# bcgsc/ntJoin

Hardware: AMD Instinct MI355X
Metric: Gbp/s minimizer-sketch+graph-build (k=32,w=1000) (higher is better)
Workload: dtype u64

## Files before the change

ntjoin_amd/csrc/graph.hip:

```cpp
#include <algorithm>
#include <cstdlib>
#include <cstring>
#include <system_error>
#include <thread>

#include "mxg_internal.h"
#include "scan_kernels.h"

namespace mxg {

static constexpr uint64_t HT_EMPTY = 0xFFFFFFFFFFFFFFFFull;
static constexpr uint32_t NONE32 = 0xFFFFFFFFu;

struct Slot {
    unsigned long long key;
    uint32_t nseen, ndup;
};

__device__ __forceinline__ uint32_t ht_slot(Slot *tab, uint32_t mask, uint32_t cap, uint64_t key)
{
    if (key == HT_EMPTY) return cap;
    uint32_t s = (uint32_t)((key * 0x9E3779B97F4A7C15ull) >> 32) & mask;
    while (true) {
        unsigned long long cur = tab[s].key;
// ... 574 lines not shown
    }
    if (n_all > skew_lim) {
        __shared__ unsigned long long skey[PJ_IPB];
        __shared__ uint32_t sitem[PJ_IPB];
        __shared__ uint8_t sasm[PJ_IPB];
        __shared__ uint32_t stab[PJ_IPB];
        __shared__ uint32_t sdup[PJ_IPB / 32];
        for (uint32_t q = threadIdx.x; q < PJ_IPB; q += PJ_BT) stab[q] = 0xFFFFFFFFu;
        for (uint32_t q = threadIdx.x; q < PJ_IPB / 32; q += PJ_BT) sdup[q] = 0;
#pragma unroll
        for (uint32_t u = 0; u < U; ++u) {
            const uint32_t q = u * PJ_BT + threadIdx.x;
            skey[q] = ((unsigned long long)rec[u].y << 32) | rec[u].x;
            sitem[q] = rec[u].z;
            sasm[q] = (uint8_t)(rec[u].w & 0xFFu);
        }
        __syncthreads();
#pragma unroll
        for (uint32_t u = 0; u < U; ++u) {
            if (!((live >> u) & 1u)) continue;
            const uint32_t q = u * PJ_BT + threadIdx.x;
            const unsigned long long key = skey[q];
            const uint32_t a = rec[u].w & 0xFFu;
            uint32_t hsl = (uint32_t)(((key + a) * 0x9E3779B97F4A7C15ull) >> 40) & (2u * PJ_IPB - 1u);
            uint32_t rep = q;
            for (;;) {
                const uint32_t sft = (hsl & 1u) * 16u;
                const uint32_t word = stab[hsl >> 1], cur = (word >> sft) & 0xFFFFu;
                if (cur == 0xFFFFu) {
                    const uint32_t want = (word & ~(0xFFFFu << sft)) | (q << sft);
                    if (atomicCAS(&stab[hsl >> 1], word, want) == word) break;
                    continue;
                }
                if (skey[cur] == key && sasm[cur] == a) {
                    rep = cur;
                    break;
                }
                hsl = (hsl + 1u) & (2u * PJ_IPB - 1u);
            }
            if (rep != q) {
                atomicOr(&sdup[rep >> 5], 1u << (rep & 31u));
                p.slot[a][rec[u].z] = (sitem[rep] << 3) | PJ_VERDICT_REF;
                live &= ~(1u << u);
            }
        }
        __syncthreads();
#pragma unroll
        for (uint32_t u = 0; u < U; ++u) {
            const uint32_t q = u * PJ_BT + threadIdx.x;
            if ((sdup[q >> 5] >> (q & 31u)) & 1u) rec[u].w |= PJ_REC_DUP;
        }
    }
    for (uint32_t b = threadIdx.x; b <= pmask; b += PJ_BT) hist[b] = 0;
    __syncthreads();
#pragma unroll
    for (uint32_t u = 0; u < U; ++u)
        if ((live >> u) & 1u) atomicAdd(&hist[pj_part(((uint64_t)rec[u].y << 32) | rec[u].x, pmask)], 1u);
    __syncthreads();
    const uint32_t P = pmask + 1, per = P >= PJ_BT ? P / PJ_BT : 1u, b0 = threadIdx.x * per;
    uint32_t cn = 0;
    if (b0 < P)
        for (uint32_t u = 0; u < per; ++u) cn += hist[b0 + u];
    uint32_t run = block_exclusive<PJ_BT / 64>(cn, sh);
    uint32_t *row = M + ((size_t)c * rows2 + row_j) * (P + 1);
    if (b0 < P)
        for (uint32_t u = 0; u < per; ++u) {
            const uint32_t cb = hist[b0 + u];
            start[b0 + u] = run;
            row[b0 + u] = run;
            hist[b0 + u] = 0;
            run += cb;
        }
    if (threadIdx.x == 0) row[P] = sh[255];
    __syncthreads();
#pragma unroll
    for (uint32_t u = 0; u < U; ++u) {
        if (!((live >> u) & 1u)) continue;
        const uint32_t b = pj_part(((uint64_t)rec[u].y << 32) | rec[u].x, pmask);
        const uint32_t pos = (uint32_t)base + start[b] + atomicAdd(&hist[b], 1u);
        recs2[pos] = rec[u];
    }
}

__global__ __launch_bounds__(256) void k_flags_pj(const AsmSet p, uint32_t *cnt, uint32_t *sup, uint64_t *mask0)
{
    const uint32_t a = asm_of_block(p, blockIdx.x);
    const uint32_t i = (blockIdx.x - p.bstart[a]) * 256u + threadIdx.x;
    bool sh = false;
    {
        const bool in = i < asm_n(p, a);
        const uint32_t lane = threadIdx.x & 63u;
        const uint64_t fb = p.fol[blockIdx.x * 4u + (threadIdx.x >> 6)];
        const uint32_t v_raw = in ? p.slot[a][i] : 0u;
        const bool isf = (fb >> lane) & 1ull;
        uint32_t v = isf ? 0u : v_raw;
        bool other = isf;
        if ((v & 7u) == PJ_VERDICT_REF) {
            v = p.slot[a][v >> 3];
            other = true;
        }
        const uint32_t lead = 63u - (uint32_t)__clzll(~fb & ((2ull << lane) - 1ull));
        const uint32_t vl = __shfl(v, lead);
        if (isf) v = vl;
        if (other) v &= MXG_MX_INALL;
        if (in) {
            sh = (v & MXG_MX_SHARED) != 0;
            p.flags[a][i] = (uint8_t)(v & 7u);
            p.shared[a][i] = sh ? 1 : 0;
        }
    }
    const uint64_t bm = __ballot(sh);
    if (a == 0 && (threadIdx.x & 63u) == 0) mask0[(blockIdx.x - p.bstart[0]) * 4u + (threadIdx.x >> 6)] = bm;
    const uint32_t c = (uint32_t)__syncthreads_count(sh ? 1 : 0);
    if (threadIdx.x == 0) count_publish(cnt + p.bstart[a], sup + sup_start(p, a), blockIdx.x - p.bstart[a], c);
}

struct VertexParams {
    const uint8_t *shared;
    const uint32_t *cnt, *sup;
    uint64_t *n_shared;
    const uint32_t *slot;
    const uint64_t *hash;
    const uint32_t *pos, *rec;
    uint32_t n;
    const uint32_t *n_ptr;
    uint32_t first;
    uint32_t *vid;
    uint64_t *vhash;
    uint32_t *vpos, *vrec;
    uint32_t *fv, *frec;
    uint32_t *ivid;
};

__global__ __launch_bounds__(256) void k_vertices(const VertexParams p)
{
    __shared__ uint32_t sh[256];
    const uint32_t i = blockIdx.x * 256u + threadIdx.x;
    const bool f = i < (p.n_ptr ? min(*p.n_ptr, p.n) : p.n) && p.shared[i];
    __shared__ uint32_t sh_before;
    if (threadIdx.x < 64) {
        const uint32_t bef = count_prefix(p.cnt, p.sup, blockIdx.x);
        if (threadIdx.x == 0) sh_before = bef;
        if (blockIdx.x + 1 == gridDim.x) {
            const uint32_t all = count_prefix(p.cnt, p.sup, (p.n + 255u) / 256u);
            if (threadIdx.x == 0) *p.n_shared = all;
        }
    }
    __syncthreads();
    const uint32_t r = sh_before + block_exclusive_256(f ? 1u : 0u, sh);
    if (!f) return;
    const uint32_t s = p.slot[i];
    uint32_t v;
    if (p.first) {
        v = r;
        p.vid[s] = v;
        p.vhash[v] = p.hash[i];
    } else {
        v = p.vid[s];
    }
    const uint32_t rec = p.rec[i];
    p.vpos[v] = p.pos[i];
    p.vrec[v] = rec;
    if (p.ivid) p.ivid[i] = v;
    p.fv[r] = v;
    p.frec[r] = rec;
}

__global__ __launch_bounds__(256) void k_block_prefix(const uint32_t *__restrict__ cnt, const uint32_t *__restrict__ sup, uint32_t n,
                                                      uint32_t *__restrict__ out)
{
    __shared__ uint32_t sh[256];
    __shared__ uint32_t sh_before;
    const uint32_t e = blockIdx.x * 256u + threadIdx.x;
    const uint32_t c = e < n ? cnt[e] : 0u;
    if (threadIdx.x < 64) {
        const uint32_t bef = count_prefix(cnt, sup, blockIdx.x * 256u);
        if (threadIdx.x == 0) sh_before = bef;
    }
    __syncthreads();
    const uint32_t r = sh_before + block_exclusive_256(c, sh);
    if (e < n) out[e] = r;
}

struct VertexPjParams {
    AsmSet as;
    const uint32_t *pos[MXG_MAX_ASSEMBLIES], *rec[MXG_MAX_ASSEMBLIES];
    const uint32_t *cnt, *sup;
    uint64_t *n_shared;
    const uint64_t *mask0;
    const uint32_t *bpref0;
    uint64_t *vhash;
    uint32_t *vpos, *vrec, *fv, *frec;
    uint32_t nvs;
    uint32_t *ivid[MXG_MAX_ASSEMBLIES];
};

__global__ __launch_bounds__(256) void k_vertices_pj(const VertexPjParams p)
{
    __shared__ uint32_t sh[256];
    __shared__ uint32_t sh_before;
    const uint32_t a = asm_of_block(p.as, blockIdx.x);
    const uint32_t blk = blockIdx.x - p.as.bstart[a], nblk = p.as.bstart[a + 1] - p.as.bstart[a];
    const uint32_t i = blk * 256u + threadIdx.x;
    const bool in = i < asm_n(p.as, a);
    const uint8_t shf = in ? p.as.shared[a][i] : (uint8_t)0;
    const uint32_t vw = in && a ? p.as.slot[a][i] : 0u;
    const uint32_t rec = in ? p.rec[a][i] : 0u, pos = in ? p.pos[a][i] : 0u;
    const uint64_t hsh = in && !a ? p.as.hash[0][i] : 0ull;
    const bool f = shf != 0;
    uint32_t v0 = 0;
    if (f && a) {
        const uint32_t i0 = vw >> 3, w = i0 >> 6;
        const uint64_t *m = p.mask0 + (w & ~3u);
        v0 = p.bpref0[i0 >> 8] + (uint32_t)__popcll(p.mask0[w] & ((1ull << (i0 & 63u)) - 1ull));
        for (uint32_t q = 0; q < (w & 3u); ++q) v0 += (uint32_t)__popcll(m[q]);
    }
    if (threadIdx.x < 64) {
        const uint32_t *cnt = p.cnt + p.as.bstart[a], *sup = p.sup + sup_start(p.as, a);
        const uint32_t bef = count_prefix(cnt, sup, blk);
        if (threadIdx.x == 0) sh_before = bef;
        if (blk + 1 == nblk) {
            const uint32_t all = count_prefix(cnt, sup, nblk);
            if (threadIdx.x == 0) p.n_shared[a] = all;
        }
    }
    __syncthreads();
    const uint32_t r = sh_before + block_exclusive_256(f ? 1u : 0u, sh);
    if (in && p.ivid[a]) p.ivid[a][i] = f ? (a ? v0 : r) : 0xFFFFFFFFu;
    if (!f) return;
    const uint32_t v = a ? v0 : r;
    if (!a) p.vhash[v] = hsh;
    const size_t o = (size_t)a * p.nvs;
    p.vpos[o + v] = pos;
    p.vrec[o + v] = rec;
    p.fv[o + r] = v;
    p.frec[o + r] = rec;
}

__global__ __launch_bounds__(256) void k_adjacency(const uint32_t *__restrict__ fv0, const uint32_t *__restrict__ frec0,
                                                   const uint64_t *__restrict__ nv_ptr, uint2 *__restrict__ adj0, uint32_t stride)
{
    const uint32_t nv = (uint32_t)*nv_ptr;
    const size_t o = (size_t)blockIdx.y * stride;
    const uint32_t *fv = fv0 + o, *frec = frec0 + o;
    const uint32_t r = blockIdx.x * 256u + threadIdx.x;
    if (r >= nv) return;
    const uint32_t rec = frec[r];
    const uint32_t nx = (r + 1 < nv && frec[r + 1] == rec) ? fv[r + 1] : NONE32;
    const uint32_t pv = (r > 0 && frec[r - 1] == rec) ? fv[r - 1] : NONE32;
    adj0[o + fv[r]] = make_uint2(nx, pv);
}

struct EdgeParams {
    const uint32_t *fv;
    const uint2 *adj;
    const uint64_t *nv_ptr;
    uint32_t nv, n_asm;
    uint8_t *eflag;
    uint32_t *bsum;
    uint32_t *bsuper;
    uint64_t *n_edges;
    uint64_t *host_ctl;
    uint32_t *eu, *ev, *esup;
    double *ew;
    double weights[MXG_MAX_ASSEMBLIES];
};

__device__ __forceinline__ uint32_t edge_mask(const EdgeParams &p, uint32_t u, uint32_t v)
{
    uint32_t m = 0;
    for (uint32_t b = 0; b < p.n_asm; ++b) {
        const uint2 q = p.adj[(size_t)b * p.nv + u];
        if (q.x == v || q.y == v) m |= 1u << b;
    }
    return m;
}

__global__ __launch_bounds__(256) void k_edge_flags(const EdgeParams p)
{
    uint64_t item = (uint64_t)blockIdx.x * 256u + threadIdx.x;
    uint8_t f = 0;
    if (item < (uint64_t)p.n_asm * p.nv) {
        uint32_t a = (uint32_t)(item / p.nv);
        uint32_t r = (uint32_t)(item % p.nv);
        if (r < (uint32_t)*p.nv_ptr) {
            const uint32_t u = p.fv[item];
            uint32_t v, m = 0;
            if (p.n_asm <= 4u) {
                uint2 q[4];
#pragma unroll
                for (uint32_t b = 0; b < 4u; ++b) q[b] = b < p.n_asm ? p.adj[(size_t)b * p.nv + u] : make_uint2(NONE32, NONE32);
                v = a == 0 ? q[0].x : a == 1 ? q[1].x : a == 2 ? q[2].x : q[3].x;
#pragma unroll
                for (uint32_t b = 0; b < 4u; ++b)
                    if (b < p.n_asm && (q[b].x == v || q[b].y == v)) m |= 1u << b;
            } else {
                v = p.adj[(size_t)a * p.nv + u].x;
                if (v != NONE32) m = edge_mask(p, u, v);
            }
            if (v != NONE32) f = ((uint32_t)__builtin_ctz(m) == a) ? (p.n_asm <= 8u ? (uint8_t)m : (uint8_t)1) : (uint8_t)0;
        }
        p.eflag[item] = f;
    }
    const uint32_t c = (uint32_t)__syncthreads_count(f);
    if (threadIdx.x == 0) count_publish(p.bsum, p.bsuper, blockIdx.x, c);
}

__global__ __launch_bounds__(256) void k_edges(const EdgeParams p, uint32_t n_items)
{
    __shared__ uint32_t sh[256];
    const uint32_t item = blockIdx.x * 256u + threadIdx.x;
    const uint32_t fb = item < n_items ? p.eflag[item] : 0u;
    const bool f = fb != 0;
    uint32_t u = 0, v = 0, m = 0;
    double wsum = 0.0;
    if (f) {
        const uint32_t a = item / p.nv;
        u = p.fv[item];
        v = p.adj[(size_t)a * p.nv + u].x;
// ... 12 lines not shown
                p.host_ctl[32] = all;
            }
            if (threadIdx.x < p.n_asm) p.host_ctl[threadIdx.x] = p.nv_ptr[threadIdx.x];
        }
    }
    __syncthreads();
    const uint32_t e = sh_before + block_exclusive_256(f ? 1u : 0u, sh);
    if (!f) return;
    p.eu[e] = u;
    p.ev[e] = v;
    p.esup[e] = m;
    p.ew[e] = wsum;
}

__global__ __launch_bounds__(256) void k_apply_msgs(const uint4 *__restrict__ msgs, uint64_t n, uint32_t stride, uint32_t *adj)
{
    const uint64_t i = (uint64_t)blockIdx.x * 256u + threadIdx.x;
    if (i >= n) return;
    const uint4 m = msgs[i];
    adj[((size_t)(m.x & 255u) * stride + m.y) * 2u + ((m.x >> 8) ? 1u : 0u)] = m.z;
}

__global__ __launch_bounds__(256) void k_iota_rows(uint32_t *a, uint32_t stride)
{
    const uint32_t i = blockIdx.x * 256u + threadIdx.x;
    if (i < stride) a[(size_t)blockIdx.y * stride + i] = i;
}

template <class T>
static int d2h(mxg_handle *h, std::vector<T> &dst, const void *src, size_t n)
{
    dst.resize(n);
    if (n) MXG_HIP(h, hipMemcpyAsync(dst.data(), src, n * sizeof(T), hipMemcpyDeviceToHost, h->stream));
    return MXG_OK;
}

__global__ __launch_bounds__(256) void k_count_unique(const uint8_t *__restrict__ flags, uint32_t n, unsigned long long *counter)
{
    uint32_t i = blockIdx.x * 256u + threadIdx.x;
    bool u = i < n && (flags[i] & MXG_MX_UNIQUE);
    uint64_t m = __ballot(u);
    if ((threadIdx.x & 63u) == 0 && m) atomicAdd(counter, (unsigned long long)__popcll(m));
}

enum CtlWord : uint32_t {
    CTL_SHARED = 0,
    CTL_EDGES = 32,
    CTL_UNIQUE = 33,
    CTL_PJ_FAIL = 34,
    CTL_WORDS = 40,
};
static_assert(CTL_SHARED + MXG_MAX_ASSEMBLIES <= CTL_EDGES, "the per-assembly counts end before the other words");

static int build_graph_impl(mxg_handle *h, const GraphCall &c, bool global_table);

int build_graph(mxg_handle *h, const GraphCall &c)
{
    h->stat_graph_join = 0;
    uint64_t how = 0;
    JoinLearnt &learnt = h->pj_learnt;
    if (!c.gb) {
        uint64_t n_mx[MXG_MAX_ASSEMBLIES];
        const uint32_t n = (uint32_t)std::min<size_t>(h->asms.size(), MXG_MAX_ASSEMBLIES);
        for (uint32_t a = 0; a < n; ++a) n_mx[a] = h->asms[a]->n_mx;
        learnt.sketches_are(JoinLearnt::signature(n, n_mx));
    }
    int rc = build_graph_impl(h, c, learnt.overflowed);
    if (rc == RC_RETRY_PJ) {
        how |= MXG_JOIN_RESIZED;
        rc = build_graph_impl(h, c, false);
    }
    if (rc == RC_RETRY_PJ) rc = RC_RETRY_GLOBAL;
    if (rc == RC_RETRY_GLOBAL) {
        how |= MXG_JOIN_GAVE_UP;
        learnt.gave_up();
        rc = build_graph_impl(h, c, true);
    }
    h->stat_graph_join |= how;
    return rc;
}

struct JoinPlan : JoinShape {
    uint32_t pj_force_fail = 0;
    uint64_t *pj_mask0 = nullptr;
    uint32_t *pj_bpref0 = nullptr;
    AsmSet as_all;
    uint32_t n_fsup = 0, n_esup = 0;
    uint32_t *fsup = nullptr, *esup = nullptr, *cnt = nullptr;
    uint32_t *M = nullptr, *cursor = nullptr;
    uint4 *recs1 = nullptr, *recs2 = nullptr;
    PjSubCaps sc;
    size_t clear_words = 0;
};

static int plan_join(mxg_handle *h, int mode, const GraphBounds *gb, bool global_table, bool split, JoinPlan &pl)
{
    const uint32_t A = (uint32_t)h->asms.size();
    if (A == 0) return set_err(h, MXG_EINVAL, "mxg_build_graph: no assemblies");
    if (A > MXG_MAX_ASSEMBLIES) return set_err(h, MXG_ELIMIT, "at most %d assemblies", MXG_MAX_ASSEMBLIES);
    pl = JoinPlan();
    JoinRequest rq;
    rq.A = A;
    for (uint32_t ai = 0; ai < A; ++ai) {
        Assembly *a = h->asms[ai];
        if (!gb && !a->has_sketch) return set_err(h, MXG_EINVAL, "assembly '%s' has no sketch (call mxg_sketch)", a->name.c_str());
        rq.n_of[ai] = gb ? gb->n_bound[ai] : a->n_mx;
    }
    rq.mode = mode;
    rq.bounds = gb != nullptr;
    rq.global_table = global_table;
    rq.split = split;
    const char *join_env = knob_raw(h, "MXG_GRAPH_JOIN");
    rq.join_global = join_env && !strcmp(join_env, "global");
    rq.force_two_level = knob_u64(h, "MXG_PJ_TWO_LEVEL", 0) != 0;
    switch (join_shape(rq, h->pj_learnt, pl)) {
    case JS_TOO_MANY_MINIMIZERS: return set_err(h, MXG_ELIMIT, "too many minimizers for one table (%llu)", (unsigned long long)pl.N);
    case JS_TOO_MANY_ITEMS: return set_err(h, MXG_ELIMIT, "graph too large for 32-bit item indices");
    case JS_OK: break;
    }
    pl.pj_force_fail = knob_u64(h, "MXG_PJ_FORCE_FAIL", 0) ? 1u : 0u;
    pl.sc.n_sub = pl.n_sub;
    for (uint32_t a = 0; a < MXG_MAX_ASSEMBLIES; ++a) pl.sc.cap[a] = pl.sub_cap[a];
    const uint64_t *const n_of = pl.n_of;
    const uint32_t nb = pl.nb, P = pl.P, P1 = pl.P1;

    if (!pl.pj) MXG_HIP(h, h->g_keys.ensure(((size_t)pl.cap + 1) * sizeof(Slot)));
    const size_t nb0 = pl.nb0, nb_all = nb;
    MXG_HIP(h, h->g_vid.ensure(pl.pj ? (nb0 + nb_all) * 4 * 8 + nb0 * 4 + 64 : ((size_t)pl.cap + 1) * 4));
    pl.pj_mask0 = h->g_vid.as<uint64_t>();
    uint64_t *const pj_fol = pl.pj_mask0 + nb0 * 4;
    pl.pj_bpref0 = reinterpret_cast<uint32_t *>(pj_fol + nb_all * 4);
    MXG_HIP(h, h->g_ctl.ensure(CTL_WORDS * 8));

    AsmSet &as_all = pl.as_all;
    as_all.n_asm = A;
    as_all.full = pl.full;
    as_all.fol = pl.pj ? pj_fol : nullptr;
    for (uint32_t a = 0; a < A; ++a) {
        Assembly *as = h->asms[a];
        MXG_HIP(h, as->d_slot.ensure(std::max<uint64_t>(n_of[a] * 4, 16)));
        MXG_HIP(h, as->d_flags.ensure(std::max<uint64_t>(n_of[a], 16)));
        MXG_HIP(h, as->d_shared.ensure(std::max<uint64_t>(n_of[a], 16)));
        as_all.n[a] = (uint32_t)n_of[a];
        as_all.n_ptr[a] = gb ? gb->n_ptr[a] : nullptr;
        as_all.hash[a] = as->d_hash.as<uint64_t>();
        as_all.slot[a] = as->d_slot.as<uint32_t>();
        as_all.flags[a] = as->d_flags.as<uint8_t>();
        as_all.shared[a] = as->d_shared.as<uint8_t>();
    }
    for (uint32_t a = A; a < MXG_MAX_ASSEMBLIES; ++a) {
        as_all.n[a] = 0;
        as_all.n_ptr[a] = nullptr;
        as_all.hash[a] = nullptr;
        as_all.slot[a] = nullptr;
        as_all.flags[a] = as_all.shared[a] = nullptr;
    }
    std::copy(pl.bstart, pl.bstart + MXG_MAX_ASSEMBLIES + 1, as_all.bstart);
    pl.n_fsup = ((nb >> SUP_SHIFT) + A + 1) * SUP_STRIDE;
    pl.n_esup = sup_words(pl.e_blocks);
    MXG_HIP(h, h->g_cnt.ensure(((size_t)pl.n_fsup + pl.n_esup + pl.n_cur + nb) * 4 + 64));
    pl.fsup = h->g_cnt.as<uint32_t>();
    pl.esup = pl.fsup + pl.n_fsup;
    pl.cnt = pl.esup + pl.n_esup + pl.n_cur;
    pl.clear_words = (size_t)pl.n_fsup + pl.n_esup + pl.n_cur;
    const bool resume = mode == GRAPH_DG_EDGES || mode == GRAPH_DG_EDGES_APPLIED;
    if (nb && !resume && pl.pj && pl.two_level) {
        const size_t n_recs = (size_t)P1 * pl.cap1;
        MXG_HIP(h, h->g_part.ensure((size_t)P1 * pl.rows2 * (P + 1) * 4 + (size_t)P1 * PJ1_CS * 4));
        MXG_HIP(h, h->g_keys.ensure(n_recs * sizeof(uint4)));
        MXG_HIP(h, h->g_recs1.ensure(n_recs * sizeof(uint4)));
        pl.M = h->g_part.as<uint32_t>();
        pl.cursor = pl.n_cur ? pl.esup + pl.n_esup : pl.M + (size_t)P1 * pl.rows2 * (P + 1);
        pl.recs1 = h->g_recs1.as<uint4>();
        pl.recs2 = h->g_keys.as<uint4>();
    }
    return MXG_OK;
}

static void launch_partition(mxg_handle *h, const JoinPlan &pl, uint32_t a_lo, uint32_t a_hi, hipStream_t st, uint32_t n_sup_clear)
{
    const uint32_t blk_lo = pl.as_all.bstart[a_lo], blk_hi = pl.as_all.bstart[a_hi];
    const uint32_t n_rows1 = (blk_hi - blk_lo + PJ_IPB / 256 - 1) / (PJ_IPB / 256);
    PjSub sub{1u, 0u, 0u, pl.cap1};
    uint32_t skew_lim = (uint32_t)std::min<uint64_t>(pl.N / pl.P1 + pl.N / pl.P1 / 32 + 2048, 0xFFFFFFFFull);
    if (pl.split) {
        sub = PjSub{pl.A, a_lo, pl.sub_off[a_lo], pl.sub_cap[a_lo]};
        skew_lim = pl.skew_lim[a_lo];
    }
    if (n_rows1)
        hipLaunchKernelGGL(k_pj1_scatter, dim3(n_rows1), dim3(PJ_BT), (size_t)pl.P1 * 8, st, pl.as_all, blk_lo, blk_hi, pl.P1 - 1, pl.cap1,
                           pl.cursor, pl.recs1, pl.fsup, n_sup_clear, sub);
    hipLaunchKernelGGL(k_pj2_bucket, dim3(sub.cap / PJ_IPB, pl.P1), dim3(PJ_BT), (size_t)pl.P * 8, st, pl.as_all, pl.recs1, pl.cursor, pl.cap1,
                       pl.rows2, pl.P - 1, pl.M, pl.recs2, knob_u64(h, "MXG_PJ_SKEW", 0) ? 0u : skew_lim, sub);
}

static int ev_pair(mxg_handle *h, hipEvent_t *a, hipEvent_t *b)
{
    while (h->ev_pool.size() < h->ev_used + 2) {
        hipEvent_t e;
        MXG_HIP(h, hipEventCreate(&e));
        h->ev_pool.push_back(e);
    }
    *a = h->ev_pool[h->ev_used];
    *b = h->ev_pool[h->ev_used + 1];
    h->ev_used += 2;
    h->ev_spans.push_back(TimedSpan{*a, *b, 0, false, 5});
    return MXG_OK;
}

int graph_plan_early(mxg_handle *h, const GraphBounds &gb, bool *early)
{
    *early = false;
    h->pj_early_done = 0;
    if (knob_u64(h, "MXG_PJ_EARLY", 1) == 0) return MXG_OK;
    MXG_HIP(h, hipSetDevice(h->device));
    if (!h->pj_plan) h->pj_plan = new JoinPlan;
    JoinPlan &pl = *h->pj_plan;
    const std::string err_before = h->err;
    if (plan_join(h, GRAPH_FULL, &gb, h->pj_learnt.overflowed, true, pl) != MXG_OK || !(pl.pj && pl.two_level && pl.split && pl.nb)) {
        pl = JoinPlan();
        h->err = err_before;
        return MXG_OK;
    }
    MXG_HIP(h, hipMemsetAsync(pl.fsup, 0, pl.clear_words * 4, h->stream));
    if (!h->ev_plan) MXG_HIP(h, hipEventCreateWithFlags(&h->ev_plan, hipEventDisableTiming));
    MXG_HIP(h, hipEventRecord(h->ev_plan, h->stream));
    *early = true;
    return MXG_OK;
}

int graph_partition_early(mxg_handle *h, uint32_t a, hipStream_t st)
// ... 14 lines not shown
    if (fine) MXG_HIP(h, hipEventRecord(e1, st));
    ++h->pj_early_done;
    return MXG_OK;
}

void graph_drop_plan(mxg_handle *h)
{
    delete h->pj_plan;
    h->pj_plan = nullptr;
}

static int take_or_make_plan(mxg_handle *h, const GraphCall &c, bool global_table, JoinPlan &own, const JoinPlan **plan)
{
    const JoinPlan *ep = h->pj_plan;
    bool early = ep && ep->split && h->pj_early_done != 0 && h->pj_early_done == ep->A && c.gb && c.mode == GRAPH_FULL && !global_table &&
                 ep->A == h->asms.size();
    for (uint32_t a = 0; early && a < ep->A; ++a) early = c.gb->n_bound[a] == ep->n_of[a] && c.gb->n_ptr[a] == ep->as_all.n_ptr[a];
    h->pj_early_done = 0;
    *plan = early ? ep : &own;
    if (early) return MXG_OK;
    const int rc = plan_join(h, c.mode, c.gb, global_table, false, own);
    if (rc != MXG_OK && c.mode != GRAPH_DG_EDGES && c.mode != GRAPH_DG_EDGES_APPLIED)
        for (Assembly *a : h->asms) a->flags_valid = a->flags_on_host = false;
    return rc;
}

struct GraphStage {
    mxg_handle *const h;
    const GraphCall &c;
    const JoinPlan &pl;
    const bool early;
    const bool resume;
    const bool fine, timing;
    Graph &g;
    uint64_t *ctl = nullptr, *hctl = nullptr;
    uint64_t *pj_fail = nullptr;

    GraphStage(mxg_handle *h_, const GraphCall &c_, const JoinPlan &pl_, bool early_)
        : h(h_), c(c_), pl(pl_), early(early_), resume(c_.mode == GRAPH_DG_EDGES || c_.mode == GRAPH_DG_EDGES_APPLIED),
          fine((h_->cfg.flags & MXG_FLAG_TIMING_FINE) != 0 && c_.mode == GRAPH_FULL), timing((h_->cfg.flags & MXG_FLAG_TIMING) != 0 || fine),
          g(h_->graph)
    {
    }
    bool joins() const { return pl.nb && !resume; }
    size_t anv() const { return (size_t)pl.A * pl.nvs; }

    int begin()
    {
        for (uint32_t ai = 0; ai < pl.A; ++ai) {
            Assembly *a = h->asms[ai];
            if (!resume) a->flags_on_host = false;
            a->flags_valid = true;
        }
        if (!resume) g = Graph();
        g.n_asm = pl.A;
        if (fine && !h->ev_g[0]) {
            MXG_HIP(h, hipEventCreate(&h->ev_g[0]));
            MXG_HIP(h, hipEventCreate(&h->ev_g[1]));
        }
        if (timing) MXG_HIP(h, hipEventRecord(h->ev0, h->stream));
        if (!resume)
            h->stat_graph_join = (pl.pj ? (pl.two_level ? MXG_JOIN_LDS_TWO_LEVEL : MXG_JOIN_LDS) : MXG_JOIN_GLOBAL) | (early ? MXG_JOIN_EARLY : 0);
        if (!pl.pj && !resume) MXG_HIP(h, hipMemsetAsync(h->g_keys.p, 0xFF, ((size_t)pl.cap + 1) * sizeof(Slot), h->stream));
        ctl = h->g_ctl.as<uint64_t>();
        if (!h->pinned_gctl) MXG_HIP(h, hipHostMalloc((void **)&h->pinned_gctl, CTL_WORDS * 8));
        hctl = h->pinned_gctl;
        memset(hctl, 0, CTL_WORDS * 8);
        pj_fail = pl.dg_pj ? dg_pj_fail_word(h) : hctl + CTL_PJ_FAIL;
        return MXG_OK;
    }

    void launch_join(uint4 *recs, uint32_t *M, uint32_t n_parts, uint32_t n_rows, const uint32_t *cursor)
    {
        const bool narrow = pl.A <= 16;
        const uint32_t cap1 = cursor ? pl.cap1 : 0u, rows2 = cursor ? pl.rows2 : 0u;
        const uint64_t pipe_blocks = cursor ? knob_u64(h, "MXG_PJ_PIPE", 1024) : 0;
        if (pipe_blocks && rows2 <= 256)
            hipLaunchKernelGGL(narrow ? k_pj_join_pipe<true> : k_pj_join_pipe<false>, dim3((uint32_t)std::min<uint64_t>(pipe_blocks, n_parts)),
                               dim3(256), 0, h->stream, recs, M, pl.P, n_parts, pj_fail, pl.pj_force_fail, cursor, cap1, rows2, pl.as_all, pl.sc);
        else
            hipLaunchKernelGGL(narrow ? k_pj_join<true> : k_pj_join<false>, dim3(n_parts), dim3(256), 0, h->stream, recs, M, pl.P, n_rows,
                               pj_fail, pl.pj_force_fail, cursor, cap1, rows2, pl.as_all, pl.sc);
    }
    int join_two_level()
    {
        if (!early) {
            MXG_HIP(h, hipMemsetAsync(pl.cursor, 0, (size_t)pl.P1 * PJ1_CS * 4, h->stream));
            launch_partition(h, pl, 0, pl.A, h->stream, pl.n_fsup + pl.n_esup);
        }
        launch_join(pl.recs2, pl.M, pl.P1 * pl.P, 0u, pl.cursor);
        hipLaunchKernelGGL(k_flags_pj, dim3(pl.nb), dim3(256), 0, h->stream, pl.as_all, pl.cnt, pl.fsup, pl.pj_mask0);
        return MXG_OK;
    }
    int join_one_level()
    {
        const uint32_t n_rows = (pl.nb + PJ_IPB / 256 - 1) / (PJ_IPB / 256);
        MXG_HIP(h, h->g_part.ensure((size_t)n_rows * (pl.P + 1) * 4));
        MXG_HIP(h, h->g_keys.ensure((size_t)n_rows * PJ_IPB * sizeof(uint4)));
        uint32_t *M = h->g_part.as<uint32_t>();
        uint4 *recs = h->g_keys.as<uint4>();
        hipLaunchKernelGGL(k_pj_bucket, dim3(n_rows), dim3(PJ_BT), (size_t)pl.P * 8, h->stream, pl.as_all, pl.nb, pl.P - 1, M, recs, pl.fsup,
                           pl.n_fsup + pl.n_esup);
        launch_join(recs, M, pl.P, n_rows, nullptr);
        hipLaunchKernelGGL(k_flags_pj, dim3(pl.nb), dim3(256), 0, h->stream, pl.as_all, pl.cnt, pl.fsup, pl.pj_mask0);
        return MXG_OK;
    }
    int join_global()
    {
        hipLaunchKernelGGL(k_insert, dim3(pl.nb), dim3(256), 0, h->stream, pl.as_all, h->g_keys.as<Slot>(), pl.mask, pl.cap, pl.fsup,
                           pl.n_fsup + pl.n_esup);
        hipLaunchKernelGGL(k_flags, dim3(pl.nb), dim3(256), 0, h->stream, pl.as_all, h->g_keys.as<Slot>(), pl.cnt, pl.fsup);
        return MXG_OK;
    }
    int mark(hipEvent_t ev)
    {
        MXG_HIP(h, hipGetLastError());
        if (fine) MXG_HIP(h, hipEventRecord(ev, h->stream));
        return MXG_OK;
    }

    int vertex_arrays()
    {
        MXG_HIP(h, h->g_vhash.ensure(pl.nvs * 8));
        MXG_HIP(h, h->g_vpos.ensure(anv() * 4));
        MXG_HIP(h, h->g_vrec.ensure(anv() * 4));
        MXG_HIP(h, h->g_fv.ensure(anv() * 4));
        MXG_HIP(h, h->g_frec.ensure(anv() * 4));
        MXG_HIP(h, h->g_nxt.ensure(2 * anv() * 4));
        if (c.mode == GRAPH_DG_EDGES) MXG_HIP(h, hipMemsetAsync(h->g_nxt.p, 0xFF, 2 * anv() * 4, h->stream));
        return MXG_OK;
    }
    int item_vids(uint32_t a, uint32_t **ivid)
    {
        *ivid = nullptr;
        if (c.mode != GRAPH_DG_VERTICES) return MXG_OK;
        MXG_HIP(h, h->asms[a]->d_ivid.ensure((size_t)pl.n_of[a] * 4 + 16));
        *ivid = h->asms[a]->d_ivid.as<uint32_t>();
        return MXG_OK;
    }
    int fill(VertexPjParams &vp)
    {
        vp.as = pl.as_all;
        for (uint32_t a = 0; a < MXG_MAX_ASSEMBLIES; ++a) {
            vp.pos[a] = a < pl.A ? h->asms[a]->d_pos.as<uint32_t>() : nullptr;
            vp.rec[a] = a < pl.A ? h->asms[a]->d_rec.as<uint32_t>() : nullptr;
            vp.ivid[a] = nullptr;
            int rc;
            if (a < pl.A && (rc = item_vids(a, &vp.ivid[a])) != MXG_OK) return rc;
        }
        vp.cnt = pl.cnt;
        vp.sup = pl.fsup;
        vp.n_shared = ctl + CTL_SHARED;
        vp.mask0 = pl.pj_mask0;
        vp.bpref0 = pl.pj_bpref0;
        vp.vhash = h->g_vhash.as<uint64_t>();
        vp.vpos = h->g_vpos.as<uint32_t>();
        vp.vrec = h->g_vrec.as<uint32_t>();
        vp.fv = h->g_fv.as<uint32_t>();
        vp.frec = h->g_frec.as<uint32_t>();
        vp.nvs = (uint32_t)pl.nvs;
        return MXG_OK;
    }
    int vertices_pj()
    {
        VertexPjParams vp;
        const int rc = fill(vp);
        if (rc != MXG_OK) return rc;
        hipLaunchKernelGGL(k_block_prefix, dim3((uint32_t)((pl.nb0 + 255) / 256)), dim3(256), 0, h->stream, pl.cnt + pl.as_all.bstart[0],
                           pl.fsup + sup_start(pl.as_all, 0), (uint32_t)pl.nb0, pl.pj_bpref0);
        hipLaunchKernelGGL(k_vertices_pj, dim3(pl.nb), dim3(256), 0, h->stream, vp);
        return MXG_OK;
    }
    int fill(VertexParams &vp, uint32_t a)
    {
        Assembly *as = h->asms[a];
        const size_t row = (size_t)a * pl.nvs;
        vp.shared = as->d_shared.as<uint8_t>();
        vp.cnt = pl.cnt + pl.as_all.bstart[a];
        vp.sup = pl.fsup + sup_start(pl.as_all, a);
        vp.n_shared = ctl + CTL_SHARED + a;
        vp.slot = as->d_slot.as<uint32_t>();
        vp.hash = as->d_hash.as<uint64_t>();
        vp.pos = as->d_pos.as<uint32_t>();
        vp.rec = as->d_rec.as<uint32_t>();
        vp.n = (uint32_t)pl.n_of[a];
        vp.n_ptr = c.gb ? c.gb->n_ptr[a] : nullptr;
        vp.first = a == 0;
        vp.vid = h->g_vid.as<uint32_t>();
        vp.vhash = h->g_vhash.as<uint64_t>();
        vp.vpos = h->g_vpos.as<uint32_t>() + row;
        vp.vrec = h->g_vrec.as<uint32_t>() + row;
        vp.fv = h->g_fv.as<uint32_t>() + row;
        vp.frec = h->g_frec.as<uint32_t>() + row;
        return item_vids(a, &vp.ivid);
    }
    int vertices_global()
    {
        for (uint32_t a = 0; a < pl.A; ++a) {
            VertexParams vp;
            const int rc = fill(vp, a);
            if (rc != MXG_OK) return rc;
            if (vp.ivid) MXG_HIP(h, hipMemsetAsync(vp.ivid, 0xFF, (size_t)vp.n * 4, h->stream));
            hipLaunchKernelGGL(k_vertices, dim3((vp.n + 255) / 256), dim3(256), 0, h->stream, vp);
        }
        return MXG_OK;
    }
    int hand_back_vertices()
    {
        g.nv_stride = pl.nvs;
        if (!c.d_n_vertices) return MXG_OK;
        if (pl.nvs > 0) MXG_HIP(h, hipMemcpyAsync(c.d_n_vertices, ctl + CTL_SHARED, 8, hipMemcpyDeviceToDevice, h->stream));
        else MXG_HIP(h, hipMemsetAsync(c.d_n_vertices, 0, 8, h->stream));
        return MXG_OK;
    }

    void adjacency_own()
    {
        hipLaunchKernelGGL(k_adjacency, dim3((uint32_t)((pl.nvs + 255) / 256), pl.A), dim3(256), 0, h->stream, h->g_fv.as<uint32_t>(),
                           h->g_frec.as<uint32_t>(), ctl + CTL_SHARED, h->g_nxt.as<uint2>(), (uint32_t)pl.nvs);
    }
    void adjacency_of_owner()
    {
        if (c.n_msgs && c.mode == GRAPH_DG_EDGES)
            hipLaunchKernelGGL(k_apply_msgs, dim3((uint32_t)((c.n_msgs + 255) / 256)), dim3(256), 0, h->stream,
                               static_cast<const uint4 *>(c.d_msgs), c.n_msgs, (uint32_t)pl.nvs, h->g_nxt.as<uint32_t>());
        hipLaunchKernelGGL(k_iota_rows, dim3((uint32_t)((pl.nvs + 255) / 256), pl.A), dim3(256), 0, h->stream, h->g_fv.as<uint32_t>(),
                           (uint32_t)pl.nvs);
    }

    void fill(EdgeParams &ep)
    {
        ep.fv = h->g_fv.as<uint32_t>();
        ep.adj = h->g_nxt.as<uint2>();
        ep.nv_ptr = ctl + CTL_SHARED;
        ep.nv = (uint32_t)pl.nvs;
        ep.n_asm = pl.A;
        ep.eflag = h->g_eflag.as<uint8_t>();
        ep.bsum = h->g_ebs.as<uint32_t>();
        ep.bsuper = pl.esup;
        ep.n_edges = ctl + CTL_EDGES;
        ep.host_ctl = hctl;
        ep.eu = h->g_eu.as<uint32_t>();
        ep.ev = h->g_ev.as<uint32_t>();
        ep.esup = h->g_esup.as<uint32_t>();
        ep.ew = h->g_ew.as<double>();
        for (uint32_t a = 0; a < MXG_MAX_ASSEMBLIES; ++a) ep.weights[a] = a < pl.A ? h->asms[a]->weight : 0.0;
    }
    int edges()
    {
        const uint32_t n_items = pl.n_items;
        MXG_HIP(h, h->g_eflag.ensure(n_items));
        MXG_HIP(h, h->g_ebs.ensure((size_t)pl.e_blocks * 4 + 64));
        MXG_HIP(h, h->g_eu.ensure((size_t)n_items * 4));
        MXG_HIP(h, h->g_ev.ensure((size_t)n_items * 4));
        MXG_HIP(h, h->g_esup.ensure((size_t)n_items * 4));
        MXG_HIP(h, h->g_ew.ensure((size_t)n_items * 8));
        EdgeParams ep;
        fill(ep);
        hipLaunchKernelGGL(k_edge_flags, dim3(pl.e_blocks), dim3(256), 0, h->stream, ep);
        hipLaunchKernelGGL(k_edges, dim3(pl.e_blocks), dim3(256), 0, h->stream, ep, n_items);
        MXG_HIP(h, hipGetLastError());
        return MXG_OK;
    }

    int sync_and_verdict()
    {
        if (timing) MXG_HIP(h, hipEventRecord(h->ev1, h->stream));
        MXG_HIP(h, stream_wait(h->stream));
        if (!pl.pj || !hctl[CTL_PJ_FAIL]) return MXG_OK;
        if (!pl.two_level || pl.pj_force_fail) return RC_RETRY_GLOBAL;
        std::vector<uint32_t> cur((size_t)pl.P1 * pl.n_sub * PJ1_CS);
        MXG_HIP(h, hipMemcpy(cur.data(), pl.cursor, cur.size() * 4, hipMemcpyDeviceToHost));
        return join_overflow_verdict(pl, cur.data(), h->pj_learnt);
    }
    int results()
    {
        const uint64_t nv = hctl[CTL_SHARED];
        for (uint32_t a = 1; a < pl.A; ++a)
            if (hctl[CTL_SHARED + a] != nv)
                return set_err(h, MXG_EDEVICE, "internal error: shared-minimizer counts differ between assemblies (%llu vs %llu)",
                               (unsigned long long)hctl[CTL_SHARED + a], (unsigned long long)nv);
        g.nv = nv;
        g.nv_stride = pl.nvs;
        g.ne = pl.nvs > 0 ? hctl[CTL_EDGES] : 0;
        h->stat_unique = ~0ull;
        if (timing) {
            float ms = 0;
            MXG_HIP(h, hipEventElapsedTime(&ms, h->ev0, h->ev1));
            h->tm.ms_graph += ms;
            if (fine && pl.nvs > 0) {
                float a = 0, b = 0, c3 = 0;
                MXG_HIP(h, hipEventElapsedTime(&a, h->ev0, h->ev_g[0]));
                MXG_HIP(h, hipEventElapsedTime(&b, h->ev_g[0], h->ev_g[1]));
                MXG_HIP(h, hipEventElapsedTime(&c3, h->ev_g[1], h->ev1));
                h->tm.ms_join += a;
                h->tm.ms_vertices += b;
                h->tm.ms_edges += c3;
            }
        }
        g.valid = true;
        g.host_valid = false;
        return MXG_OK;
    }
};

static int build_graph_impl(mxg_handle *h, const GraphCall &c, bool global_table)
{
    MXG_HIP(h, hipSetDevice(h->device));
    JoinPlan own;
    const JoinPlan *plan = nullptr;
    int rc = take_or_make_plan(h, c, global_table, own, &plan);
    if (rc != MXG_OK) return rc;
    const JoinPlan &pl = *plan;
    GraphStage s(h, c, pl, plan != &own);
    if ((rc = s.begin()) != MXG_OK) return rc;
    if (s.joins() && (rc = pl.pj ? (pl.two_level ? s.join_two_level() : s.join_one_level()) : s.join_global()) != MXG_OK) return rc;
    if ((rc = s.mark(h->ev_g[0])) != MXG_OK) return rc;
    if (pl.nvs > 0) {
        if ((rc = s.vertex_arrays()) != MXG_OK) return rc;
        if (!s.resume && (rc = pl.pj ? s.vertices_pj() : s.vertices_global()) != MXG_OK) return rc;
    }
    if (c.mode == GRAPH_DG_VERTICES) return s.hand_back_vertices();
    if (pl.nvs > 0) {
        if (c.mode == GRAPH_FULL) s.adjacency_own();
        else s.adjacency_of_owner();
        if ((rc = s.mark(h->ev_g[1])) != MXG_OK) return rc;
        if ((rc = s.edges()) != MXG_OK) return rc;
    }
    if ((rc = s.sync_and_verdict()) != MXG_OK) return rc;
    return s.results();
}

int graph_to_host(mxg_handle *h)
{
    Graph &g = h->graph;
    if (!g.valid) return set_err(h, MXG_EINVAL, "call mxg_build_graph first");
    if (g.host_valid) return MXG_OK;
    MXG_HIP(h, hipSetDevice(h->device));
    const size_t anv = (size_t)g.n_asm * g.nv;
    int rc;
    {
        std::vector<std::thread> th;
        auto sized = [](auto &v, size_t n) {
            try {
                v.resize(n);
            } catch (const std::bad_alloc &) {
            }
        };
        try {
            th.emplace_back([&] { sized(g.vhash, g.nv); });
            th.emplace_back([&] { sized(g.vpos, anv); });
            th.emplace_back([&] { sized(g.vrec, anv); });
            th.emplace_back([&] { sized(g.eu, g.ne); });
            th.emplace_back([&] { sized(g.ev, g.ne); });
            th.emplace_back([&] { sized(g.esup, g.ne); });
            sized(g.ew, g.ne);
        } catch (const std::system_error &) {
        }
        for (auto &t : th) t.join();
    }
    if ((rc = d2h(h, g.vhash, h->g_vhash.p, g.nv)) != MXG_OK) return rc;
    g.vpos.resize(anv);
    g.vrec.resize(anv);
    for (uint32_t a = 0; a < g.n_asm && g.nv; ++a) {
        MXG_HIP(h, hipMemcpyAsync(g.vpos.data() + (size_t)a * g.nv, h->g_vpos.as<uint32_t>() + (size_t)a * g.nv_stride,
                                  g.nv * 4, hipMemcpyDeviceToHost, h->stream));
        MXG_HIP(h, hipMemcpyAsync(g.vrec.data() + (size_t)a * g.nv, h->g_vrec.as<uint32_t>() + (size_t)a * g.nv_stride,
                                  g.nv * 4, hipMemcpyDeviceToHost, h->stream));
    }
    if ((rc = d2h(h, g.eu, h->g_eu.p, g.ne)) != MXG_OK) return rc;
    if ((rc = d2h(h, g.ev, h->g_ev.p, g.ne)) != MXG_OK) return rc;
    if ((rc = d2h(h, g.esup, h->g_esup.p, g.ne)) != MXG_OK) return rc;
    if ((rc = d2h(h, g.ew, h->g_ew.p, g.ne)) != MXG_OK) return rc;
    MXG_HIP(h, hipStreamSynchronize(h->stream));
    g.host_valid = true;
    return MXG_OK;
}

int flags_to_host(mxg_handle *h, Assembly *a)
{
    if (!a->flags_valid) return set_err(h, MXG_EINVAL, "call mxg_build_graph first");
    if (a->flags_on_host) return MXG_OK;
    MXG_HIP(h, hipSetDevice(h->device));
    int rc = d2h(h, a->h_flags, a->d_flags.p, a->n_mx);
    if (rc != MXG_OK) return rc;
    MXG_HIP(h, hipStreamSynchronize(h->stream));
    a->flags_on_host = true;
    return MXG_OK;
}

}
```

Baseline: 2504.

## Fuse adjacency into vertex kernel and widen flags kernel to four items per thread

The flags kernel now handles four minimizers per thread with vectorized slot loads and packed flag stores. It builds per-block shared masks for every assembly, so the per-item shared byte array is no longer written. The vertex kernel reads sharedness from those masks. In full-graph mode it also computes next/previous neighbours in shared memory, using cross-block searches for the nearest shared item, which removes the separate adjacency kernel and the frec array. This cuts memory traffic and a kernel launch, at the cost of more complex boundary logic and extra wave work in the vertex kernel.

```diff
diff --git a/ntjoin_amd/csrc/graph.hip b/ntjoin_amd/csrc/graph.hip
--- a/ntjoin_amd/csrc/graph.hip
+++ b/ntjoin_amd/csrc/graph.hip
@@ -680,37 +680,104 @@
     }
 }
 
-__global__ __launch_bounds__(256) void k_flags_pj(const AsmSet p, uint32_t *cnt, uint32_t *sup, uint64_t *mask0)
-{
-    const uint32_t a = asm_of_block(p, blockIdx.x);
-    const uint32_t i = (blockIdx.x - p.bstart[a]) * 256u + threadIdx.x;
-    bool sh = false;
-    {
-        const bool in = i < asm_n(p, a);
-        const uint32_t lane = threadIdx.x & 63u;
-        const uint64_t fb = p.fol[blockIdx.x * 4u + (threadIdx.x >> 6)];
-        const uint32_t v_raw = in ? p.slot[a][i] : 0u;
-        const bool isf = (fb >> lane) & 1ull;
-        uint32_t v = isf ? 0u : v_raw;
-        bool other = isf;
-        if ((v & 7u) == PJ_VERDICT_REF) {
-            v = p.slot[a][v >> 3];
-            other = true;
-        }
-        const uint32_t lead = 63u - (uint32_t)__clzll(~fb & ((2ull << lane) - 1ull));
-        const uint32_t vl = __shfl(v, lead);
-        if (isf) v = vl;
-        if (other) v &= MXG_MX_INALL;
-        if (in) {
-            sh = (v & MXG_MX_SHARED) != 0;
-            p.flags[a][i] = (uint8_t)(v & 7u);
-            p.shared[a][i] = sh ? 1 : 0;
-        }
-    }
-    const uint64_t bm = __ballot(sh);
-    if (a == 0 && (threadIdx.x & 63u) == 0) mask0[(blockIdx.x - p.bstart[0]) * 4u + (threadIdx.x >> 6)] = bm;
-    const uint32_t c = (uint32_t)__syncthreads_count(sh ? 1 : 0);
-    if (threadIdx.x == 0) count_publish(cnt + p.bstart[a], sup + sup_start(p, a), blockIdx.x - p.bstart[a], c);
+__device__ __forceinline__ uint64_t spread16_by4(uint64_t x)
+{
+    x &= 0xFFFFull;
+    x = (x | (x << 24)) & 0x000000FF000000FFull;
+    x = (x | (x << 12)) & 0x000F000F000F000Full;
+    x = (x | (x << 6)) & 0x0303030303030303ull;
+    x = (x | (x << 3)) & 0x1111111111111111ull;
+    return x;
+}
+template <uint32_t IPT>
+__host__ __device__ __forceinline__ uint32_t flags_pj_tiles(const AsmSet &p, uint32_t a)
+{
+    return (p.bstart[a + 1] - p.bstart[a] + IPT - 1u) / IPT;
+}
+
+template <uint32_t IPT>
+__global__ __launch_bounds__(256) void k_flags_pj(const AsmSet p, uint32_t *cnt, uint32_t *sup, uint64_t *mask)
+{
+    static_assert(IPT == 1 || IPT == 4, "a thread's minimizers lie in one follower word; a 256-block is a wave (4) or the block (1)");
+    __shared__ uint32_t lv[256 * IPT];
+    uint32_t a = 0, tile = blockIdx.x;
+    for (;;) {
+        const uint32_t nt = flags_pj_tiles<IPT>(p, a);
+        if (a + 1 >= p.n_asm || tile < nt) break;
+        tile -= nt;
+        ++a;
+    }
+    const uint32_t nblk = p.bstart[a + 1] - p.bstart[a], n = asm_n(p, a);
+    const uint32_t t0 = threadIdx.x * IPT, i0 = tile * (256u * IPT) + t0;
+    const uint32_t blk = i0 >> 8, bit0 = i0 & 63u;
+    const bool blk_in = blk < nblk;
+    const size_t w = ((size_t)p.bstart[a] + blk) * 4u + ((i0 >> 6) & 3u);
+    const uint64_t fb = blk_in ? p.fol[w] : 0ull;
+    uint32_t v[IPT];
+    bool whole = false;
+    if constexpr (IPT == 4) {
+        whole = i0 + 4u <= n;
+        if (whole) {
+            const uint4 q = *reinterpret_cast<const uint4 *>(p.slot[a] + i0);
+            v[0] = q.x, v[1] = q.y, v[2] = q.z, v[3] = q.w;
+        }
+    }
+    if (!whole) {
+#pragma unroll
+        for (uint32_t j = 0; j < IPT; ++j) v[j] = i0 + j < n ? p.slot[a][i0 + j] : 0u;
+    }
+    uint32_t other = 0;
+#pragma unroll
+    for (uint32_t j = 0; j < IPT; ++j) {
+        const bool isf = (fb >> (bit0 + j)) & 1ull;
+        if (isf) {
+            v[j] = 0u;
+            other |= 1u << j;
+        }
+        if ((v[j] & 7u) == PJ_VERDICT_REF) {
+            v[j] = p.slot[a][v[j] >> 3];
+            other |= 1u << j;
+        }
+        lv[t0 + j] = v[j];
+    }
+    __syncthreads();
+    uint32_t fl = 0, shm = 0;
+#pragma unroll
+    for (uint32_t j = 0; j < IPT; ++j) {
+        const uint32_t bit = bit0 + j;
+        if ((fb >> bit) & 1ull)
+            v[j] = lv[(t0 & ~63u) + 63u - (uint32_t)__clzll(~fb & ((2ull << bit) - 1ull))];
+        if ((other >> j) & 1u) v[j] &= MXG_MX_INALL;
+        if (i0 + j < n) {
+            fl |= (v[j] & 7u) << (8u * j);
+            shm |= ((v[j] & MXG_MX_SHARED) ? 1u : 0u) << j;
+        }
+    }
+    if (whole) {
+        *reinterpret_cast<uint32_t *>(p.flags[a] + i0) = fl;
+    } else {
+#pragma unroll
+        for (uint32_t j = 0; j < IPT; ++j)
+            if (i0 + j < n) p.flags[a][i0 + j] = (uint8_t)(fl >> (8u * j));
+    }
+    const uint32_t lane = threadIdx.x & 63u;
+    if constexpr (IPT == 4) {
+        uint64_t mw = 0;
+        uint32_t c = 0;
+#pragma unroll
+        for (uint32_t j = 0; j < IPT; ++j) {
+            const uint64_t b = __ballot((shm >> j) & 1u);
+            mw |= spread16_by4(b >> (lane & 48u)) << j;
+            c += (uint32_t)__popcll(b);
+        }
+        if (blk_in && (lane & 15u) == 0) mask[w] = mw;
+        if (blk_in && lane == 0) count_publish(cnt + p.bstart[a], sup + sup_start(p, a), blk, c);
+    } else {
+        const uint64_t bm = __ballot(shm & 1u);
+        if (lane == 0) mask[w] = bm;
+        const uint32_t c = (uint32_t)__syncthreads_count(shm & 1u);
+        if (threadIdx.x == 0) count_publish(cnt + p.bstart[a], sup + sup_start(p, a), blk, c);
+    }
 }
 
 struct VertexParams {
@@ -785,54 +852,115 @@
     const uint32_t *pos[MXG_MAX_ASSEMBLIES], *rec[MXG_MAX_ASSEMBLIES];
     const uint32_t *cnt, *sup;
     uint64_t *n_shared;
-    const uint64_t *mask0;
+    const uint64_t *mask;
     const uint32_t *bpref0;
     uint64_t *vhash;
-    uint32_t *vpos, *vrec, *fv, *frec;
+    uint32_t *vpos, *vrec, *fv;
+    uint2 *adj;
     uint32_t nvs;
     uint32_t *ivid[MXG_MAX_ASSEMBLIES];
 };
 
+__device__ __forceinline__ uint32_t pj_vertex_of(const VertexPjParams &p, uint32_t i0)
+{
+    const uint32_t w = i0 >> 6;
+    const uint64_t *m = p.mask + (w & ~3u);
+    uint32_t v0 = p.bpref0[i0 >> 8] + (uint32_t)__popcll(p.mask[w] & ((1ull << (i0 & 63u)) - 1ull));
+    for (uint32_t q = 0; q < (w & 3u); ++q) v0 += (uint32_t)__popcll(m[q]);
+    return v0;
+}
+
+__device__ __forceinline__ uint32_t pj_shared_before(const uint32_t *cnt, const uint64_t *mask, uint32_t blk, bool far)
+{
+    const uint32_t lane = threadIdx.x & 63u;
+    for (uint32_t hi = blk; hi > 0; hi = hi > 64u ? hi - 64u : 0u) {
+        const uint64_t some = __ballot(lane < hi && cnt[hi - 1u - (lane < hi ? lane : 0u)] != 0u);
+        if (some) {
+            const uint32_t b = hi - 1u - (uint32_t)__builtin_ctzll(some);
+            const uint64_t m = mask[(size_t)b * 4u + (lane & 3u)];
+            const uint32_t q = 31u - (uint32_t)__builtin_clz((uint32_t)__ballot(m != 0ull) & 15u);
+            return b * 256u + q * 64u + 63u - (uint32_t)__clzll(__shfl(m, (int)q));
+        }
+        if (!far) break;
+    }
+    return NONE32;
+}
+__device__ __forceinline__ uint32_t pj_shared_after(const uint32_t *cnt, const uint64_t *mask, uint32_t blk, uint32_t nblk, bool far)
+{
+    const uint32_t lane = threadIdx.x & 63u;
+    for (uint32_t lo = blk + 1u; lo < nblk; lo += 64u) {
+        const uint64_t some = __ballot(lo + lane < nblk && cnt[lo + lane < nblk ? lo + lane : lo] != 0u);
+        if (some) {
+            const uint32_t b = lo + (uint32_t)__builtin_ctzll(some);
+            const uint64_t m = mask[(size_t)b * 4u + (lane & 3u)];
+            const uint32_t q = (uint32_t)__builtin_ctz((uint32_t)__ballot(m != 0ull) & 15u);
+            return b * 256u + q * 64u + (uint32_t)__builtin_ctzll(__shfl(m, (int)q));
+        }
+        if (!far) break;
+    }
+    return NONE32;
+}
+
 __global__ __launch_bounds__(256) void k_vertices_pj(const VertexPjParams p)
 {
     __shared__ uint32_t sh[256];
     __shared__ uint32_t sh_before;
+    __shared__ uint32_t nb_v[258], nb_rec[258];
     const uint32_t a = asm_of_block(p.as, blockIdx.x);
     const uint32_t blk = blockIdx.x - p.as.bstart[a], nblk = p.as.bstart[a + 1] - p.as.bstart[a];
-    const uint32_t i = blk * 256u + threadIdx.x;
+    const uint32_t i = blk * 256u + threadIdx.x, wave = threadIdx.x >> 6, lane = threadIdx.x & 63u;
     const bool in = i < asm_n(p.as, a);
-    const uint8_t shf = in ? p.as.shared[a][i] : (uint8_t)0;
+    const bool f = (p.mask[(size_t)blockIdx.x * 4u + wave] >> lane) & 1ull;
     const uint32_t vw = in && a ? p.as.slot[a][i] : 0u;
     const uint32_t rec = in ? p.rec[a][i] : 0u, pos = in ? p.pos[a][i] : 0u;
     const uint64_t hsh = in && !a ? p.as.hash[0][i] : 0ull;
-    const bool f = shf != 0;
-    uint32_t v0 = 0;
-    if (f && a) {
-        const uint32_t i0 = vw >> 3, w = i0 >> 6;
-        const uint64_t *m = p.mask0 + (w & ~3u);
-        v0 = p.bpref0[i0 >> 8] + (uint32_t)__popcll(p.mask0[w] & ((1ull << (i0 & 63u)) - 1ull));
-        for (uint32_t q = 0; q < (w & 3u); ++q) v0 += (uint32_t)__popcll(m[q]);
-    }
-    if (threadIdx.x < 64) {
-        const uint32_t *cnt = p.cnt + p.as.bstart[a], *sup = p.sup + sup_start(p.as, a);
+    const uint32_t v0 = f && a ? pj_vertex_of(p, vw >> 3) : 0u;
+    const uint32_t *cnt = p.cnt + p.as.bstart[a];
+    uint32_t out_v = NONE32, out_rec = 0, out_i = NONE32;
+    if (wave == 0) {
+        const uint32_t *sup = p.sup + sup_start(p.as, a);
         const uint32_t bef = count_prefix(cnt, sup, blk);
         if (threadIdx.x == 0) sh_before = bef;
         if (blk + 1 == nblk) {
             const uint32_t all = count_prefix(cnt, sup, nblk);
             if (threadIdx.x == 0) p.n_shared[a] = all;
         }
+    } else if (wave <= 2 && p.adj) {
+        const uint64_t *mask = p.mask + (size_t)p.as.bstart[a] * 4u;
+        const bool far = cnt[blk] != 0u;
+        out_i = wave == 1 ? pj_shared_before(cnt, mask, blk, far) : pj_shared_after(cnt, mask, blk, nblk, far);
+        if (out_i != NONE32) {
+            out_rec = p.rec[a][out_i];
+            if (a) out_v = pj_vertex_of(p, p.as.slot[a][out_i] >> 3);
+        }
     }
     __syncthreads();
-    const uint32_t r = sh_before + block_exclusive_256(f ? 1u : 0u, sh);
-    if (in && p.ivid[a]) p.ivid[a][i] = f ? (a ? v0 : r) : 0xFFFFFFFFu;
+    const uint32_t q = block_exclusive_256(f ? 1u : 0u, sh), r = sh_before + q;
+    const uint32_t v = a ? v0 : r;
+    if (in && p.ivid[a]) p.ivid[a][i] = f ? v : 0xFFFFFFFFu;
+    const size_t o = (size_t)a * p.nvs;
+    if (f) {
+        if (!a) p.vhash[v] = hsh;
+        p.vpos[o + v] = pos;
+        p.vrec[o + v] = rec;
+        p.fv[o + r] = v;
+    }
+    if (!p.adj) return;
+    const uint32_t total = sh[255];
+    if (f) {
+        nb_v[1u + q] = v;
+        nb_rec[1u + q] = rec;
+    }
+    if ((wave == 1 || wave == 2) && lane == 0) {
+        const uint32_t at = wave == 1 ? 0u : 1u + total;
+        nb_v[at] = out_i == NONE32 ? NONE32 : a ? out_v : wave == 1 ? sh_before - 1u : sh_before + total;
+        nb_rec[at] = out_rec;
+    }
+    __syncthreads();
     if (!f) return;
-    const uint32_t v = a ? v0 : r;
-    if (!a) p.vhash[v] = hsh;
-    const size_t o = (size_t)a * p.nvs;
-    p.vpos[o + v] = pos;
-    p.vrec[o + v] = rec;
-    p.fv[o + r] = v;
-    p.frec[o + r] = rec;
+    const uint32_t nx = nb_rec[2u + q] == rec ? nb_v[2u + q] : NONE32;
+    const uint32_t pv = nb_rec[q] == rec ? nb_v[q] : NONE32;
+    p.adj[o + v] = make_uint2(nx, pv);
 }
 
 __global__ __launch_bounds__(256) void k_adjacency(const uint32_t *__restrict__ fv0, const uint32_t *__restrict__ frec0,
@@ -1011,7 +1139,7 @@
 
 struct JoinPlan : JoinShape {
     uint32_t pj_force_fail = 0;
-    uint64_t *pj_mask0 = nullptr;
+    uint64_t *pj_mask = nullptr;
     uint32_t *pj_bpref0 = nullptr;
     AsmSet as_all;
     uint32_t n_fsup = 0, n_esup = 0;
@@ -1055,9 +1183,9 @@
 
     if (!pl.pj) MXG_HIP(h, h->g_keys.ensure(((size_t)pl.cap + 1) * sizeof(Slot)));
     const size_t nb0 = pl.nb0, nb_all = nb;
-    MXG_HIP(h, h->g_vid.ensure(pl.pj ? (nb0 + nb_all) * 4 * 8 + nb0 * 4 + 64 : ((size_t)pl.cap + 1) * 4));
-    pl.pj_mask0 = h->g_vid.as<uint64_t>();
-    uint64_t *const pj_fol = pl.pj_mask0 + nb0 * 4;
+    MXG_HIP(h, h->g_vid.ensure(pl.pj ? (nb_all + nb_all) * 4 * 8 + nb0 * 4 + 64 : ((size_t)pl.cap + 1) * 4));
+    pl.pj_mask = h->g_vid.as<uint64_t>();
+    uint64_t *const pj_fol = pl.pj_mask + nb_all * 4;
     pl.pj_bpref0 = reinterpret_cast<uint32_t *>(pj_fol + nb_all * 4);
     MXG_HIP(h, h->g_ctl.ensure(CTL_WORDS * 8));
 
@@ -1069,13 +1197,13 @@
         Assembly *as = h->asms[a];
         MXG_HIP(h, as->d_slot.ensure(std::max<uint64_t>(n_of[a] * 4, 16)));
         MXG_HIP(h, as->d_flags.ensure(std::max<uint64_t>(n_of[a], 16)));
-        MXG_HIP(h, as->d_shared.ensure(std::max<uint64_t>(n_of[a], 16)));
+        if (!pl.pj) MXG_HIP(h, as->d_shared.ensure(std::max<uint64_t>(n_of[a], 16)));
         as_all.n[a] = (uint32_t)n_of[a];
         as_all.n_ptr[a] = gb ? gb->n_ptr[a] : nullptr;
         as_all.hash[a] = as->d_hash.as<uint64_t>();
         as_all.slot[a] = as->d_slot.as<uint32_t>();
         as_all.flags[a] = as->d_flags.as<uint8_t>();
-        as_all.shared[a] = as->d_shared.as<uint8_t>();
+        as_all.shared[a] = pl.pj ? nullptr : as->d_shared.as<uint8_t>();
     }
     for (uint32_t a = A; a < MXG_MAX_ASSEMBLIES; ++a) {
         as_all.n[a] = 0;
@@ -1256,6 +1384,12 @@
             hipLaunchKernelGGL(narrow ? k_pj_join<true> : k_pj_join<false>, dim3(n_parts), dim3(256), 0, h->stream, recs, M, pl.P, n_rows,
                                pj_fail, pl.pj_force_fail, cursor, cap1, rows2, pl.as_all, pl.sc);
     }
+    void launch_flags_pj()
+    {
+        uint32_t tiles = 0;
+        for (uint32_t a = 0; a < pl.A; ++a) tiles += flags_pj_tiles<4>(pl.as_all, a);
+        hipLaunchKernelGGL(k_flags_pj<4>, dim3(tiles), dim3(256), 0, h->stream, pl.as_all, pl.cnt, pl.fsup, pl.pj_mask);
+    }
     int join_two_level()
     {
         if (!early) {
@@ -1263,7 +1397,7 @@
             launch_partition(h, pl, 0, pl.A, h->stream, pl.n_fsup + pl.n_esup);
         }
         launch_join(pl.recs2, pl.M, pl.P1 * pl.P, 0u, pl.cursor);
-        hipLaunchKernelGGL(k_flags_pj, dim3(pl.nb), dim3(256), 0, h->stream, pl.as_all, pl.cnt, pl.fsup, pl.pj_mask0);
+        launch_flags_pj();
         return MXG_OK;
     }
     int join_one_level()
@@ -1276,7 +1410,7 @@
         hipLaunchKernelGGL(k_pj_bucket, dim3(n_rows), dim3(PJ_BT), (size_t)pl.P * 8, h->stream, pl.as_all, pl.nb, pl.P - 1, M, recs, pl.fsup,
                            pl.n_fsup + pl.n_esup);
         launch_join(recs, M, pl.P, n_rows, nullptr);
-        hipLaunchKernelGGL(k_flags_pj, dim3(pl.nb), dim3(256), 0, h->stream, pl.as_all, pl.cnt, pl.fsup, pl.pj_mask0);
+        launch_flags_pj();
         return MXG_OK;
     }
     int join_global()
@@ -1299,7 +1433,7 @@
         MXG_HIP(h, h->g_vpos.ensure(anv() * 4));
         MXG_HIP(h, h->g_vrec.ensure(anv() * 4));
         MXG_HIP(h, h->g_fv.ensure(anv() * 4));
-        MXG_HIP(h, h->g_frec.ensure(anv() * 4));
+        if (!pl.pj && !resume) MXG_HIP(h, h->g_frec.ensure(anv() * 4));
         MXG_HIP(h, h->g_nxt.ensure(2 * anv() * 4));
         if (c.mode == GRAPH_DG_EDGES) MXG_HIP(h, hipMemsetAsync(h->g_nxt.p, 0xFF, 2 * anv() * 4, h->stream));
         return MXG_OK;
@@ -1325,13 +1459,13 @@
         vp.cnt = pl.cnt;
         vp.sup = pl.fsup;
         vp.n_shared = ctl + CTL_SHARED;
-        vp.mask0 = pl.pj_mask0;
+        vp.mask = pl.pj_mask;
         vp.bpref0 = pl.pj_bpref0;
         vp.vhash = h->g_vhash.as<uint64_t>();
         vp.vpos = h->g_vpos.as<uint32_t>();
         vp.vrec = h->g_vrec.as<uint32_t>();
         vp.fv = h->g_fv.as<uint32_t>();
-        vp.frec = h->g_frec.as<uint32_t>();
+        vp.adj = c.mode == GRAPH_FULL ? h->g_nxt.as<uint2>() : nullptr;
         vp.nvs = (uint32_t)pl.nvs;
         return MXG_OK;
     }
@@ -1496,8 +1630,8 @@
     }
     if (c.mode == GRAPH_DG_VERTICES) return s.hand_back_vertices();
     if (pl.nvs > 0) {
-        if (c.mode == GRAPH_FULL) s.adjacency_own();
-        else s.adjacency_of_owner();
+        if (c.mode != GRAPH_FULL) s.adjacency_of_owner();
+        else if (!pl.pj) s.adjacency_own();
         if ((rc = s.mark(h->ev_g[1])) != MXG_OK) return rc;
         if ((rc = s.edges()) != MXG_OK) return rc;
     }
```

After: 2548, median of 4. 1.02x the previous value.
